# patrickfrey/strusPattern

Measured on AMD Instinct MI355X. Metric: GB/s input text scanned + matches/s, 10k-regex lexer + 10k-rule automaton, higher is better.
Workload: dtype u64; 1 GPU; configs[4] per-GPU shard: 10001 regexes + 10000 token rules, 12288 docs x 64KiB UTF-8 per step (the same 805 MB resident in HBM every step; configs[4] asks 32 GB per GPU: 39 such steps)

## Files before the change

### struspattern_amd/csrc/l2_fast.h

```cpp
#ifndef SPA_L2_FAST_H
#define SPA_L2_FAST_H
#include <stdint.h>
#include <string>
#include <vector>
#include "l2_tables.h"
#include "l2_device.h"

namespace spa {

struct FastKeyInst
{
	uint32_t resultHandle;
	uint32_t formatHandle;
	uint32_t pastEvent;
	uint32_t meta;
	struct { uint32_t event; uint32_t info; } trig[ 3];
	uint32_t hw0;
	uint32_t ranksA;
	uint32_t ranksB;
	uint32_t totals;
	uint32_t items;
	uint32_t flags;
};
enum {
// ... 68 lines not shown
	{
		s.count = 0; s.value = 0; s.flags |= S_DEL;
		return;
	}
	if (took)
	{
		if ((info & FTI_HASVAR) && withItems)
		{
			const uint32_t item = elex | ((info >> FTI_VAR_SHIFT) << 24);
			if ((s.flags & S_DONE) && !(s.flags & S_HASLIST)) {}
			else if (s.nItems == 0) { s.it0 = item; s.nItems = 1; }
			else if (s.nItems == 1) { s.it1 = item; s.nItems = 2; }
			else if (s.nItems == 2) { s.it2 = item; s.nItems = 3; }
			else s.flags |= S_ODD;
		}
		if (!(s.flags & S_HASSTART)) { s.startLex = elex; s.flags |= S_TOOK; if (esord) s.flags |= S_HASSTART; }
	}
	if (m)
	{
		if (!(s.flags & S_DONE)) { s.flags |= S_DONE | S_RESULT; if (s.nItems) s.flags |= S_HASLIST; }
		if (f) s.flags |= S_FIN;
	}
}

struct FastKeyEntry
{
	uint32_t event;
	uint32_t kiBegin;
	uint32_t kiCount;
	uint32_t stopIdx;
};

enum {FAST_LISTCAP=64, FAST_EXPCAP=1024, FAST_MAXSTOP=64, FAST_SPILL_BUCKET=1024, FAST_VARIANTS=5, FAST_RQCAP=192};

struct FastSpillLayout
{
	uint32_t maxRules;
	uint32_t oCold;
	uint32_t oHot, oLink;
	uint32_t oKi, oLex0;
	uint32_t oFree;
	uint32_t oEnt;
	uint32_t oStaged;
	uint32_t maxStaged;
	uint32_t oList;
	uint32_t oExp;
	uint32_t totalWords;
};

enum {SPD_FAST_FALLBACK=100};

struct FastParams
{
	const FastKeyInst* keyinst;
	const FastStatic* statics;
	const FastKeyEntry* keytab;
	uint32_t keymask;
	uint32_t nofStopWords;
	uint32_t expShift;
	uint32_t bucketMeta[ 16];
	FastSpillLayout spill;
	uint32_t* spillBase;
	uint32_t* fallbackList; uint32_t* fallbackCount;
	uint32_t* diag;
	L2BatchIO io;
	uint64_t* prof;
// ... 15 lines not shown
```

### struspattern_amd/csrc/l2_fast_kernel.hip

```cpp
#include <hip/hip_runtime.h>
#include <stdint.h>
#include "l2_fast.h"
#include "l2_device.h"
#include "wave_scan.h"

using namespace spa;

namespace {

typedef uint16_t u16;
typedef uint8_t u8;

typedef const __attribute__((address_space(4))) FastParams& KP;
__device__ __forceinline__ KP kernelParams() { return *(const __attribute__((address_space(4))) FastParams*)__builtin_amdgcn_kernarg_segment_ptr(); }

#define WAVE_FENCE() __builtin_amdgcn_fence( __ATOMIC_ACQ_REL, "wavefront")

enum {NIL16=0xFFFFu};

#ifdef SPA_PROF
#define PROF_DECL u64 prof_t0 = __builtin_amdgcn_s_memtime()
#define PROF_ADD( SLOT) do { const u64 prof_t1 = __builtin_amdgcn_s_memtime(); w.prof[ SLOT] += prof_t1 - prof_t0; prof_t0 = prof_t1; } while (0)
#else
#define PROF_DECL do {} while (0)
// ... 40 lines not shown
{
	const u32 inc = 1u << ((h & 3u)*8), ws = h >> 2;
	c0 += ws == 0 ? inc : 0u; c1 += ws == 1 ? inc : 0u; c2 += ws == 2 ? inc : 0u; c3 += ws == 3 ? inc : 0u;
}

#define FALLBACK( WHY) do { w.err = SPD_FAST_FALLBACK; w.why = (WHY); } while (0)
enum {FB_LEXEMS=1, FB_DISPOSE=2, FB_ITEM_AFTER_RESULT=3, FB_ITEMS=4, FB_STAGED=5, FB_RULES=8, FB_BUCKET_SIZE=9, FB_POSLEXEMS=10};

__device__ __forceinline__ bool endLE( u32 hw, u32 pos) { return (hw & H_ENDZERO) || ((hw >> H_END_SHIFT) & H_END_MASK) != ((pos + 1u) & 0xFFu); }
__device__ __forceinline__ bool endEQ( u32 hw, u32 pos) { return (hw & H_ENDZERO) ? (pos == 0) : (((hw >> H_END_SHIFT) & H_END_MASK) == (pos & 0xFFu)); }
__device__ __forceinline__ u32 withEnd( u32 hw, u32 end) { return (hw & ~((H_END_MASK << H_END_SHIFT) | H_ENDZERO)) | ((end & 0xFFu) << H_END_SHIFT); }

template <bool SMALL> struct FreeId { typedef u8 type; };
template <> struct FreeId<false> { typedef u16 type; };
template <int R, int T>
struct LdsDoc
{
	u32 hot[ R];
	u32 kl[ R];
	u64 ent[ T];
	u32 bsize[ 16];
	u32 bmeta[ 16];
	u16 link[ 3*R];
	typename FreeId<(R <= 256)>::type freeS[ R];
	u16 exp[ FAST_EXPCAP];
	u16 expCnt[ 64];
	u16 list[ FAST_LISTCAP];
	u16 rq[ FAST_RQCAP];
};

struct Wave
{
	u32* sp;
	u32 curpos, timestamp, nInstalled, nAlt, nSignals, nTrig, openLo, openHi;
	u32 freeN, usedL, sFreeN, usedS;
	u32 nDispose, nStaged, nStagedItems, err;
	u32 lbase;
	u32 spill;
	u32 why;
	u32 posLexems;
	u32 stopLex, stopOrd, stopTs;
	u32 bsizeV, bmetaV;
	u32 expCntV;
#ifdef SPA_PROF
	u64 prof[ 12];
#endif
};

template <int R, int T>
struct Engine
{
typedef LdsDoc<R,T> Lds;
typedef __attribute__((address_space(3))) Lds& LR;

template <bool SP> static __device__ __forceinline__ u32 ldHot( LR L, const Wave& w, KP P, u32 r) { if (!SP || r < (u32)R) return L.hot[ r]; return w.sp[ P.spill.oHot + (r - R)]; }
template <bool SP> static __device__ __forceinline__ void stHot( LR L, const Wave& w, KP P, u32 r, u32 v) { if (!SP || r < (u32)R) L.hot[ r] = v; else w.sp[ P.spill.oHot + (r - R)] = v; }
template <bool SP> static __device__ __forceinline__ u32 ldLink( LR L, const Wave& w, KP P, u32 r, u32 j) { if (!SP || r < (u32)R) return (u32)L.link[ 3*r + j]; return w.sp[ P.spill.oLink + 3*(r - R) + j]; }
template <bool SP> static __device__ __forceinline__ void stLink( LR L, const Wave& w, KP P, u32 r, u32 j, u32 v) { if (!SP || r < (u32)R) L.link[ 3*r + j] = (u16)v; else w.sp[ P.spill.oLink + 3*(r - R) + j] = v; }
template <bool SP> static __device__ __forceinline__ void ldLinks( LR L, const Wave& w, KP P, u32 r, u32& l0, u32& l1, u32& l2)
{
	if (!SP || r < (u32)R) { l0 = (u32)L.link[ 3*r]; l1 = (u32)L.link[ 3*r+1]; l2 = (u32)L.link[ 3*r+2]; }
	else { const u32* q = &w.sp[ P.spill.oLink + 3*(r - R)]; l0 = q[0]; l1 = q[1]; l2 = q[2]; }
}
template <bool SP> static __device__ __forceinline__ u32 ldKl( LR L, const Wave& w, KP P, u32 r) { if (!SP || r < (u32)R) return L.kl[ r]; return w.sp[ P.spill.oKi + (r - R)]; }
template <bool SP> static __device__ __forceinline__ void stKl( LR L, const Wave& w, KP P, u32 r, u32 ki, u32 lx)
{ const u32 v = ki | (lx << 20); if (!SP || r < (u32)R) L.kl[ r] = v; else w.sp[ P.spill.oKi + (r - R)] = v; }
static __device__ __forceinline__ u32 keyLexemOf( u32 kl, u32 lbase) { return lbase - ((lbase - (kl >> 20)) & 0xFFFu); }
template <bool SP> static __device__ __forceinline__ u32 ldExp( LR L, const Wave& w, KP P, u32 row, u32 i)
{ const u32 C = (u32)FAST_EXPCAP >> P.expShift; if (!SP || i < C) return (u32)L.exp[ row*C + i]; return w.sp[ P.spill.oExp + row*P.spill.maxRules + (i - C)]; }
template <bool SP> static __device__ __forceinline__ void stExp( LR L, const Wave& w, KP P, u32 row, u32 i, u32 r)
{ const u32 C = (u32)FAST_EXPCAP >> P.expShift; if (!SP || i < C) L.exp[ row*C + i] = (u16)r; else w.sp[ P.spill.oExp + row*P.spill.maxRules + (i - C)] = r; }
template <bool SP> static __device__ __forceinline__ u32 ldEv( LR L, const Wave& w, KP P, u32 h, u32 meta, u32 pos)
{ if (!SP || pos < (meta >> 16)) return (u32)L.ent[ (meta & 0xFFFFu) + pos]; return w.sp[ P.spill.oEnt + 2*(h*FAST_SPILL_BUCKET + pos - (meta >> 16))]; }
template <bool SP> static __device__ __forceinline__ uint2 ldEnt( LR L, const Wave& w, KP P, u32 h, u32 meta, u32 pos)
{ if (!SP || pos < (meta >> 16)) { const u64 v = L.ent[ (meta & 0xFFFFu) + pos]; return make_uint2( (u32)v, (u32)(v >> 32)); } return *(const uint2*)&w.sp[ P.spill.oEnt + 2*(h*FAST_SPILL_BUCKET + pos - (meta >> 16))]; }
template <bool SP> static __device__ __forceinline__ u32 ldTs( LR L, const Wave& w, KP P, u32 h, u32 meta, u32 pos) { return ldEnt<SP>( L, w, P, h, meta, pos).y; }
template <bool SP> static __device__ __forceinline__ void stEnt( LR L, const Wave& w, KP P, u32 h, u32 meta, u32 pos, u32 e, u32 t)
{
	if (!SP || pos < (meta >> 16)) L.ent[ (meta & 0xFFFFu) + pos] = (u64)e | ((u64)t << 32);
	else *(uint2*)&w.sp[ P.spill.oEnt + 2*(h*FAST_SPILL_BUCKET + pos - (meta >> 16))] = make_uint2( e, t);
}
template <bool SP> static __device__ __forceinline__ u32 ldList( LR L, const Wave& w, KP P, u32 i) { if (!SP || i < (u32)FAST_LISTCAP) return (u32)L.list[ i]; return w.sp[ P.spill.oList + i]; }
static __device__ __forceinline__ void pushList( LR L, Wave& w, KP P, u32 i, u32 r)
{
	if (i < (u32)FAST_LISTCAP) { if (LANE == 0) L.list[ i] = (u16)r; }
	else { w.spill = 1; if (LANE == 0) w.sp[ P.spill.oList + i] = r; }
}

enum {STAGED_LINE=0x80000000u};
static __device__ __forceinline__ void stageLineResult( Wave& w, KP P, u32 at, u32 ki, u32 startLex, u32 endLex, u32 nStatic, u32 hasNew, u32 newVar, u32 keyLex)
{
	u32* S = &w.sp[ P.spill.oStaged + 8*at];
	st4( S, (u32)STAGED_LINE | ki, 0u, startLex, endLex);
	*(uint2*)(S+4) = make_uint2( nStatic | (hasNew << 2) | (newVar << 8), keyLex);
}
static __device__ __forceinline__ void stageResult( Wave& w, KP P, u32 at, u32 handle, u32 fmt, u32 startLex, u32 endLex, u32 nItems, u32 vars, u32 i0, u32 i1, u32 i2)
{
	u32* S = &w.sp[ P.spill.oStaged + 8*at];
	st4( S, handle, fmt, startLex, endLex);
	st4( S+4, nItems | (vars << 8), i0, i1, i2);
}

template <bool SP>
static __device__ __forceinline__ void fireSignal( LR L, Wave& w, KP P, u32 tsv, u32 sord)
{
	const u32 tid = tsv & 0xFFFFu, r = tid >> 2;
	const u32 sigval = (tsv >> 16) & 0xFu, sigtype = (tsv >> 20) & 0x7u, hasVar = (tsv >> 23) & 1u, variable = tsv >> 24;
	u32 hw = uni( ldHot<SP>( L, w, P, r));
	w.nSignals += 1;
	u32 value = hw & H_VALUE_MASK, count = (hw >> H_COUNT_SHIFT) & H_COUNT_MASK;
	bool match = false, take = false, fin = false;
	switch (sigtype)
	{
		case SIG_ANY:
			take = true;
			if (count > 0) { match = true; --count; fin = (count == 0); hw = withEnd( hw, sord+1); }
			break;
		case SIG_SEQUENCE:
		case SIG_SEQUENCE_IMM:
			if (sigval == value && (sigtype == SIG_SEQUENCE ? endLE( hw, sord) : endEQ( hw, sord)))
			{
				hw = withEnd( hw, sord+1); value = sigval-1;
				if (count > 0) { --count; match = (count == 0); } else match = true;
				fin = (value == 0); take = true;
			}
			break;
		case SIG_WITHIN:
			if ((sigval & value) != 0 && endLE( hw, sord))
			{
				hw = withEnd( hw, sord+1); value &= ~sigval;
				if (count > 0) { --count; match = (count == 0); } else match = true;
				take = true;
			}
			break;
		default:
			hw &= ~(H_VALUE_MASK | (H_COUNT_MASK << H_COUNT_SHIFT));
			if (!(hw & H_LISTED))
			{
				if (w.nDispose < P.spill.maxRules) { pushList( L, w, P, w.nDispose, r); w.nDispose += 1; hw |= H_LISTED; } else FALLBACK( FB_DISPOSE);
			}
			if (LANE == 0) stHot<SP>( L, w, P, r, hw);
			return;
// ... 157 lines not shown
			handle = c0.x; fmt = c0.y; startLex = c0.z; it0 = c0.w; it1 = c1.x; it2 = c1.y;
		}
		else
		{
			const u32* K = (const u32*)&P.keyinst[ kl & 0xFFFFFu];
			handle = K[ 0]; fmt = K[ 1];
			const u32 vars = K[ 14];
			startLex = lx;
			it0 = lx | ((vars & 0xFFu) << 24); it1 = lx | (((vars >> 8) & 0xFFu) << 24); it2 = lx | (((vars >> 16) & 0xFFu) << 24);
		}
		if (newItem)
		{
			const u32 item = w.lbase | (variable << 24);
			if (nItems == 0) it0 = item; else if (nItems == 1) it1 = item; else it2 = item;
			nItemsOut = nItems + 1u;
		}
		if (newStart) startLex = w.lbase;
	}
	else if (lineCase && newItem) nItemsOut = nItems + 1u;
	const bool resLine = lineCase && (hw & H_VISIBLE) != 0, resRec = recCase && match && handle != 0;
	const u64 resM = __ballot( resLine || resRec);
	const u32 nres = (u32)__popcll( resM);
	const bool listNow = hit && !(hw & H_LISTED) && (isDel || (match && fin));
	const u64 listM = __ballot( listNow);
	const u32 nlist = (u32)__popcll( listM);
	{
		const u64 whyM = __ballot( why != 0);
		u32 fb = 0;
		if (whyM) fb = (u32)__builtin_amdgcn_readlane( why, (u32)__builtin_ctzll( whyM));
		else if (w.nStaged + nres > P.spill.maxStaged) fb = FB_STAGED;
		else if (w.nDispose + nlist > P.spill.maxRules) fb = FB_DISPOSE;
		if (fb) { FALLBACK( fb); return true; }
	}
	w.nSignals += nh;
	if (nres)
	{
		const u32 at = w.nStaged + (u32)__popcll( resM & lanesBelow());
		if (resLine) stageLineResult( w, P, at, kl & 0xFFFFFu, newStart ? w.lbase : lx, w.lbase, nItems, newItem ? 1u : 0u, variable, lx);
		if (resRec)
		{
			const u32 ia = nItemsOut == 3 ? it2 : nItemsOut == 2 ? it1 : it0;
			const u32 ib = nItemsOut == 3 ? it1 : it0;
			const u32 ic = it0;
			const u32 vars = nItemsOut == 0 ? 0u : nItemsOut == 1 ? (ia >> 24) : nItemsOut == 2 ? ((ia >> 24) | ((ib >> 24) << 8)) : ((ia >> 24) | ((ib >> 24) << 8) | ((ic >> 24) << 16));
			stageResult( w, P, at, handle, fmt, startLex, w.lbase, nItemsOut, vars, ia & 0xFFFFFFu, ib & 0xFFFFFFu, ic & 0xFFFFFFu);
		}
		w.nStaged += nres;
		const u32 itemsIncl = waveScanAdd( (resLine || resRec) ? nItemsOut : 0u);
		w.nStagedItems += (u32)__builtin_amdgcn_readlane( itemsIncl, 63);
	}
	if (recCase && !match)
	{
		st4( cold, handle, fmt, startLex, it0); *(uint2*)(cold + 4) = make_uint2( it1, it2);
		hw |= H_COLD;
	}
	if (nlist)
	{
		if (listNow) L.list[ w.nDispose + (u32)__popcll( listM & lanesBelow())] = (u16)r;
		w.nDispose += nlist;
	}
	if (hit)
	{
		if (listNow) hw |= H_LISTED;
		if (!isDel)
		{
			if (newStart && sord) hw |= H_HASSTART;
			hw = (hw & ~(H_VALUE_MASK | (H_COUNT_MASK << H_COUNT_SHIFT) | (H_NITEMS_MASK << H_NITEMS_SHIFT))) | value | (count << H_COUNT_SHIFT) | ((live ? nItemsOut : nItems) << H_NITEMS_SHIFT);
// ... 18 lines not shown
#if defined(SPA_PROF) && !defined(SPA_PROF_INSTALL)
		u64 pd0 = __builtin_amdgcn_s_memtime();
#define PROF_D( SLOT) do { if (__ballot( hw == 0xFFFFFFFFu)) w.err = SPD_ERR_INTERNAL; const u64 pd1 = __builtin_amdgcn_s_memtime(); w.prof[ SLOT] += pd1 - pd0; pd0 = pd1; } while (0)
#else
#define PROF_D( SLOT) do {} while (0)
#endif
		if (have)
		{
			r = isExp ? ldExp<SP>( L, w, P, row, nE - 1u - (base + LANE - nD)) : ldList<SP>( L, w, P, base + LANE);
			hw = ldHot<SP>( L, w, P, r);
		}
		const bool act = have && (hw & H_ACTIVE) && !(isExp && (hw & H_LISTED));
		const u32 mask = act ? ((hw >> H_TMASK_SHIFT) & H_TMASK_MASK) : 0u;
		if (act) stHot<SP>( L, w, P, r, hw & ~(H_ACTIVE | (H_TMASK_MASK << H_TMASK_SHIFT)));
		if (__ballot( mask != 0))
		{
			u32 lk[ 3] = {0,0,0};
			if (mask) ldLinks<SP>( L, w, P, r, lk[ 0], lk[ 1], lk[ 2]);
#if defined(SPA_PROF) && !defined(SPA_PROF_INSTALL)
			if (__ballot( lk[ 0] == 0xFFFFFFFFu)) w.err = SPD_ERR_INTERNAL;
#endif
			PROF_D( 6);
			const bool slot2 = __ballot( (mask & 4u) != 0) != 0;
			u32 c0 = 0, c1 = 0, c2 = 0, c3 = 0;
#pragma unroll
			for (int j=0; j<2; ++j) if ((mask >> j) & 1u) byteInc( c0, c1, c2, c3, lk[ j] >> 12);
			if (slot2) { if (mask & 4u) byteInc( c0, c1, c2, c3, lk[ 2] >> 12); }
			const u32 i0 = waveScanAdd( c0), i1 = waveScanAdd( c1), i2 = waveScanAdd( c2), i3 = waveScanAdd( c3);
			const u32 e0 = i0 - c0, e1 = i1 - c1, e2 = i2 - c2, e3 = i3 - c3;
			const u32 t0 = (u32)__builtin_amdgcn_readlane( i0, 63), t1 = (u32)__builtin_amdgcn_readlane( i1, 63);
			const u32 t2 = (u32)__builtin_amdgcn_readlane( i2, 63), t3 = (u32)__builtin_amdgcn_readlane( i3, 63);
			const u32 tot = LANE < 16u ? byteField( t0, t1, t2, t3, LANE) : 0u;
			const u32 qoff = waveScanAdd( tot) - tot;
			const u32 total = (u32)__builtin_amdgcn_readlane( qoff + tot, 15);
			if (slot2)
			{
				const u32 h = lk[ 2] >> 12;
				const u32 qo = (u32)__builtin_amdgcn_ds_bpermute( (int)(h << 2), (int)qoff);
				if (mask & 4u) L.rq[ qo + byteField( e0, e1, e2, e3, h)] = (u16)(4u*r + 2u);
			}
#pragma unroll
			for (int j=1; j>=0; --j)
			{
				const u32 h = lk[ j] >> 12;
				const u32 qo = (u32)__builtin_amdgcn_ds_bpermute( (int)(h << 2), (int)qoff);
				if ((mask >> j) & 1u)
				{
					u32 mineBefore = 0;
					if (slot2 && (mask & 4u) && (lk[ 2] >> 12) == h) ++mineBefore;
					if (j == 0 && (mask & 2u) && (lk[ 1] >> 12) == h) ++mineBefore;
					L.rq[ qo + byteField( e0, e1, e2, e3, h) + mineBefore] = (u16)(4u*r + (u32)j);
				}
			}
			WAVE_FENCE();
			PROF_D( 7);
			if (LANE < 16u && tot)
			{
				const u32 h = LANE, meta = w.bmetaV;
				u32 size = w.bsizeV;
				u32 tidNext = (u32)L.rq[ qoff];
				for (u32 q=0; q<tot; ++q)
				{
					const u32 tid = tidNext;
					{ const u32 nx = qoff + q + 1u; tidNext = (u32)L.rq[ nx < (u32)FAST_RQCAP ? nx : (u32)FAST_RQCAP - 1u]; }
					const u32 pos = ldLink<SP>( L, w, P, tid >> 2, tid & 3u) & 0xFFFu;
					const u32 last = size - 1u;
					const uint2 m = ldEnt<SP>( L, w, P, h, meta, last);
					if (!SP || pos != last)
					{
						stEnt<SP>( L, w, P, h, meta, pos, m.x, m.y);
						stLink<SP>( L, w, P, (m.y & 0xFFFFu) >> 2, m.y & 3u, (h << 12) | pos);
					}
					size = last;
					if (SP) WAVE_FENCE();
				}
				L.bsize[ h] = size;
				w.bsizeV = size;
			}
			WAVE_FENCE();
			PROF_D( 11);
			w.nTrig -= total;
#ifdef SPA_PROF
			w.prof[ 8] += (u32)__builtin_amdgcn_readlane( waveScanMax( tot), 63); w.prof[ 9] += 1; w.prof[ 10] += nb;
#endif
		}
		if (nE)
		{
			const bool fr = have && isExp;
			const u64 mL = __ballot( fr && r < (u32)R);
			if (fr && r < (u32)R) L.freeS[ w.freeN + (u32)__popcll( mL & lanesBelow())] = (typename FreeId<(R <= 256)>::type)r;
			w.freeN += (u32)__popcll( mL);
			if (SP)
			{
				const u64 mS = __ballot( fr && r >= (u32)R);
				if (fr && r >= (u32)R) w.sp[ P.spill.oFree + w.sFreeN + (u32)__popcll( mS & lanesBelow())] = r - R;
				w.sFreeN += (u32)__popcll( mS);
			}
		}
		WAVE_FENCE();
	}
}

static __device__ __forceinline__ void setCurrentPos( LR L, Wave& w, KP P, u32 pos)
{
	const u32 W = 1u << P.expShift;
	u32 wcnt = 0;
	while (!w.err)
	{
		u32 n = 0, row = 0;
		while (wcnt < W && w.curpos < pos && !n)
		{
			row = w.curpos & (W-1u);
			n = (u32)__builtin_amdgcn_readlane( w.expCntV, row);
			++wcnt; ++w.curpos;
// ... 59 lines not shown
	for (int j=0; j<3; ++j)
	{
		hB[ j] = (tInfo[ j] >> FTI_BUCKET_SHIFT) & 15u;
		inst[ j] = mat && (tInfo[ j] & FTI_INSTALL);
		if (inst[ j]) byteInc( c0, c1, c2, c3, hB[ j]);
	}
	u32 tmask = 0;
	if (__ballot( inst[ 0] || inst[ 1] || inst[ 2]))
	{
		u32 i0 = waveScanAdd( c0), i1 = waveScanAdd( c1), i2 = waveScanAdd( c2), i3 = waveScanAdd( c3);
		const u32 e0 = i0 - c0, e1 = i1 - c1, e2 = i2 - c2, e3 = i3 - c3;
		const u32 t0 = (u32)__builtin_amdgcn_readlane( i0, 63), t1 = (u32)__builtin_amdgcn_readlane( i1, 63);
		const u32 t2 = (u32)__builtin_amdgcn_readlane( i2, 63), t3 = (u32)__builtin_amdgcn_readlane( i3, 63);
		u32 oldSize = 0, add = 0;
		if (LANE < 16u) { oldSize = L.bsize[ LANE]; add = byteField( t0, t1, t2, t3, LANE); }
#pragma unroll
		for (int j=0; j<3; ++j)
		{
			if (inst[ j])
			{
				const u32 h = hB[ j];
				u32 sameB = 0;
#pragma unroll
				for (int jj=0; jj<j; ++jj) if (inst[ jj] && hB[ jj] == h) ++sameB;
				const u32 pos = L.bsize[ h] + byteField( e0, e1, e2, e3, h) + sameB;
				const u32 sv = (tInfo[ j] & FTI_SIGVAL_MASK) | (((tInfo[ j] >> FTI_SIGTYPE_SHIFT) & FTI_SIGTYPE_MASK) << 4) | ((tInfo[ j] & FTI_HASVAR) ? 0x80u : 0u);
				stEnt<SP>( L, w, P, h, L.bmeta[ h], pos, tEv[ j], (4*r + (u32)j) | (sv << 16) | ((tInfo[ j] >> FTI_VAR_SHIFT) << 24));
				stLink<SP>( L, w, P, r, (u32)j, (h << 12) | pos);
				tmask |= 1u << j;
			}
		}
		WAVE_FENCE();
		if (LANE < 16u && add) L.bsize[ LANE] = oldSize + add;
		{
			const u32 s = t0 + t1 + t2 + t3;
			w.nTrig += (s & 0xFFu) + ((s >> 8) & 0xFFu) + ((s >> 16) & 0xFFu) + (s >> 24);
		}
	}
	if (mat)
	{
		u32 hw = value | (count << H_COUNT_SHIFT) | H_ACTIVE | H_COLD | (tmask << H_TMASK_SHIFT) | (nItems << H_NITEMS_SHIFT);
		hw |= end ? ((end & 0xFFu) << H_END_SHIFT) : (u32)H_ENDZERO;
		if (done) hw |= H_DONE;
		if (hasStart) hw |= H_HASSTART;
		if (del || fin) hw |= H_LISTED;
		stHot<SP>( L, w, P, r, hw);
		u32* cold = &w.sp[ P.spill.oCold + 8*r];
		st4( cold, handle, fmt, startLex, it0);
		*(uint2*)(cold + 4) = make_uint2( it1, it2);
	}
	{
		const bool emit = have && resultNow && handle != 0;
		const u64 rm = __ballot( emit);
		if (rm)
		{
			const u32 nr = (u32)__popcll( rm);
			if (w.nStaged + nr > P.spill.maxStaged) { FALLBACK( FB_STAGED); return; }
			if (emit)
			{
				const u32 ia = nItems == 3 ? it2 : nItems == 2 ? it1 : it0;
				const u32 ib = nItems == 3 ? it1 : it0;
				const u32 ic = it0;
				const u32 vars = nItems == 0 ? 0u : nItems == 1 ? (ia >> 24) : nItems == 2 ? ((ia >> 24) | ((ib >> 24) << 8)) : ((ia >> 24) | ((ib >> 24) << 8) | ((ic >> 24) << 16));
				stageResult( w, P, w.nStaged + (u32)__popcll( rm & lanesBelow()), handle, fmt, startLex, w.lbase, nItems, vars, ia & 0xFFFFFFu, ib & 0xFFFFFFu, ic & 0xFFFFFFu);
			}
			w.nStaged += nr;
			u32 incl = waveScanAdd( emit ? nItems : 0u);
			w.nStagedItems += (u32)__builtin_amdgcn_readlane( incl, 63);
		}
	}
// ... 60 lines not shown
		}
		u32 hw = (hw0 & ~(H_NITEMS_MASK << H_NITEMS_SHIFT)) | (nItems << H_NITEMS_SHIFT);
		hw |= (fl & FKF_END_SET) ? (((sord + 1u) & 0xFFu) << H_END_SHIFT) : (u32)H_ENDZERO;
		stHot<SP>( L, w, P, r, hw);
		stKl<SP>( L, w, P, r, ki0 + LANE, w.lbase);
	}
	const u32 nres = (totals >> 16) & 0xFFu;
	if (nres)
	{
		if (w.nStaged + nres > P.spill.maxStaged) { FALLBACK( FB_STAGED); return; }
		if (have && (fl & FKF_RESULT_NOW))
		{
			const u32 v0 = q3.z & 0xFFu, v1 = (q3.z >> 8) & 0xFFu, v2 = (q3.z >> 16) & 0xFFu;
			const u32 va = nItems == 3 ? v2 : nItems == 2 ? v1 : v0;
			const u32 vb = nItems == 3 ? v1 : v0;
			const u32 vars = nItems == 0 ? 0u : nItems == 1 ? va : nItems == 2 ? (va | (vb << 8)) : (va | (vb << 8) | (v0 << 16));
			stageResult( w, P, w.nStaged + ((ranksA >> 16) & 0xFFu), handle, fmt, (fl & FKF_START_SET) ? w.lbase : 0u, w.lbase, nItems, vars, w.lbase, w.lbase, w.lbase);
		}
		w.nStaged += nres;
		if (P.io.withItems) w.nStagedItems += itemsTotal;
	}
	const u32 nd = totals >> 24;
	if (nd)
	{
		if (w.nDispose + nd > P.spill.maxRules) { FALLBACK( FB_DISPOSE); return; }
		if (w.nDispose + nd > (u32)FAST_LISTCAP) w.spill = 1;
		if (have && (fl & FKF_DISPOSE_NOW))
		{
			const u32 at = w.nDispose + (ranksA >> 24);
			if (at < (u32)FAST_LISTCAP) L.list[ at] = (u16)r; else w.sp[ P.spill.oList + at] = r;
		}
		w.nDispose += nd;
	}
	w.nTrig += totals & 0xFFu;
	WAVE_FENCE();
}

static __device__ __forceinline__ bool allocRuleIds( LR L, Wave& w, KP P, u64 matMask, u32& r)
{
	const bool mat = (matMask >> LANE) & 1ull;
	const u32 nmat = (u32)__popcll( matMask);
	const u32 rank = (u32)__popcll( matMask & lanesBelow());
	r = 0;
	if (nmat)
	{
		const u32 a = w.freeN < nmat ? w.freeN : nmat;
		const u32 roomL = (u32)R - w.usedL;
		const u32 b = (nmat - a) < roomL ? (nmat - a) : roomL;
		const u32 rest = nmat - a - b;
		if (rest)
		{
			const u32 c = w.sFreeN < rest ? w.sFreeN : rest;
			const u32 d = rest - c;
			if ((u32)R + w.usedS + d > P.spill.maxRules) { FALLBACK( FB_RULES); return false; }
			w.spill = 1;
			if (mat && rank >= a+b)
			{
				if (rank < a+b+c) r = (u32)R + w.sp[ P.spill.oFree + w.sFreeN - 1 - (rank - a - b)];
				else r = (u32)R + w.usedS + (rank - a - b - c);
			}
			w.sFreeN -= c; w.usedS += d;
		}
		if (mat)
		{
			if (rank < a) r = (u32)L.freeS[ w.freeN - 1 - rank];
			else if (rank < a+b) r = w.usedL + (rank - a);
		}
// ... 58 lines not shown
	const u32 nItems = P.io.withItems ? ((hw0 >> H_NITEMS_SHIFT) & H_NITEMS_MASK) : 0u;
	if (have)
	{
		const u32 close = (misc >> FSM_EXPCLOSE_SHIFT) & 0xFFu;
		if (close) L.expCnt[ row] = (u16)(cnt + close);
#pragma unroll
		for (int t=0; t<2; ++t) if (info[ t] & FSI_LAST) L.bsize[ (info[ t] >> FSI_BUCKET_SHIFT) & 15u] = oldB[ t] + ((info[ t] >> FSI_RANK_SHIFT) & 0xFFu) + 1u;
		u32 hw = (hw0 & ~(H_NITEMS_MASK << H_NITEMS_SHIFT)) | (nItems << H_NITEMS_SHIFT);
		hw |= (misc & FSM_END_SET) ? (((sord + 1u) & 0xFFu) << H_END_SHIFT) : (u32)H_ENDZERO;
		stHot<SP>( L, w, P, r, hw);
		stKl<SP>( L, w, P, r, ki0 + LANE, w.lbase);
	}
	const u32 nres = (totals >> 16) & 0xFFu;
	if (nres)
	{
		if (w.nStaged + nres > P.spill.maxStaged) { FALLBACK( FB_STAGED); return; }
		if (have && (misc & FSM_RESULT_NOW))
			stageLineResult( w, P, w.nStaged + (ranks & 0xFFu), ki0 + LANE, (misc & FSM_START_SET) ? w.lbase : 0u, w.lbase, nItems, 0u, 0u, w.lbase);
		w.nStaged += nres;
		if (P.io.withItems) w.nStagedItems += itemsTotal;
	}
	const u32 nd = totals >> 24;
	if (nd)
	{
		if (w.nDispose + nd > P.spill.maxRules) { FALLBACK( FB_DISPOSE); return; }
		if (w.nDispose + nd > (u32)FAST_LISTCAP) w.spill = 1;
		if (have && (misc & FSM_DISPOSE_NOW))
		{
			const u32 at = w.nDispose + ((ranks >> 8) & 0xFFu);
			if (at < (u32)FAST_LISTCAP) L.list[ at] = (u16)r; else w.sp[ P.spill.oList + at] = r;
		}
		w.nDispose += nd;
	}
	w.nTrig += totals & 0xFFu;
	w.nSignals += (totals >> 8) & 0xFFu;
	WAVE_FENCE();
}

static __device__ __forceinline__ void installBatch( LR L, Wave& w, KP P, u32 kb, u32 kc, u32 sord, const uint4 pc0, const uint4 pc1)
{
	for (u32 base=0; base<kc && !w.err; base+=64)
	{
		const u32 nb = (kc - base) < 64u ? (kc - base) : 64u;
		const bool have = LANE < nb;
		uint4 c0 = pc0, c1 = pc1;
		if (base)
		{
			c0 = make_uint4( 0,0,0,0); c1 = c0;
			if (have) { const u32* S = (const u32*)&P.statics[ kb + base + LANE]; c0 = ld4( S); c1 = ld4( S+4); }
		}
#ifdef SPA_PROF_INSTALL
		u64 pi0 = __builtin_amdgcn_s_memtime();
#define PROF_I( SLOT, V) do { if (__ballot( (V) == 0xFFFFFFF1u)) w.err = SPD_ERR_INTERNAL; const u64 pi1 = __builtin_amdgcn_s_memtime(); w.prof[ SLOT] += pi1 - pi0; pi0 = pi1; } while (0)
#else
#define PROF_I( SLOT, V) do {} while (0)
#endif
		if ((uni( c1.y) & FSM_BATCH_COMPACT) && sord != 0)
		{
			PROF_I( 6, c1.y);
			const u32 info[ 2] = {c0.y, c0.w};
			const u32 row = (sord + (c1.y & FSM_RANGE_MASK)) & ((1u << P.expShift) - 1u);
			u32 cnt = 0, oldB[ 2] = {0,0}, metaB[ 2] = {0,0};
			bool inst[ 3] = {false,false,false}; u32 hB[ 3] = {0,0,0};
			if (have)
			{
				cnt = (u32)L.expCnt[ row];
#pragma unroll
				for (int t=0; t<2; ++t)
// ... 52 lines not shown
#pragma unroll
					for (int j=2; j>=0; --j)
					{
						if ((tInfo[ j] & FTI_INSTALL) && tEv[ j] == pastEvent) fireLocal( sim, tInfo[ j], psord, plex, P.io.withItems);
					}
					bool cancelled = false;
#pragma unroll
					for (int j=0; j<3; ++j)
					{
						if ((tInfo[ j] & FTI_INSTALL) && ((tInfo[ j] >> FTI_SIGTYPE_SHIFT) & FTI_SIGTYPE_MASK) == SIG_DEL)
						{
							const u32 ts = delTs[ j];
							if (ts && ts > pts) cancelled = true;
						}
					}
					if (cancelled || (sim.flags & (S_DEL | S_FIN))) dropped = true;
				}
			}
			w.nAlt += (u32)__popcll( __ballot( have && pastEvent != 0));
		}
		if (!isStatic)
		{
			if (have && !dropped)
			{
#pragma unroll
				for (int j=0; j<3; ++j) if (tInfo[ j] & FTI_KEY) fireLocal( sim, tInfo[ j], sord, w.lbase, P.io.withItems);
			}
			if (__ballot( (sim.flags & S_ODD) != 0)) { FALLBACK( FB_ITEMS); return; }
		}
		const bool mat = have && !dropped;
		const u64 matMask = __ballot( mat);
		const u32 nmat = (u32)__popcll( matMask);
		w.nInstalled += nb;
		if (isStatic) w.nSignals += (uni( q3.y) >> 8) & 0xFFu;
		else
		{
			u32 incl = waveScanAdd( have ? sim.nFires : 0u);
			w.nSignals += (u32)__builtin_amdgcn_readlane( incl, 63);
		}
		u32 r;
		if (!allocRuleIds( L, w, P, matMask, r)) return;
		if (nmat && !w.spill)
		{
			const u32 row = (sord + range) & ((1u << P.expShift) - 1u);
			const bool over = mat && (u32)L.expCnt[ row] + nmat > ((u32)FAST_EXPCAP >> P.expShift);
			if (__ballot( over)) w.spill = 1;
		}
		{
			bool inst[ 3]; u32 hB[ 3];
#pragma unroll
			for (int j=0; j<3; ++j) { inst[ j] = mat && (tInfo[ j] & FTI_INSTALL); hB[ j] = (tInfo[ j] >> FTI_BUCKET_SHIFT) & 15u; }
			if (!checkBuckets( L, w, P, isStatic ? (uni( q3.y) & 0xFFu) : 3*nmat, inst, hB)) return;
		}
		if (isStatic)
		{
			if (w.spill) installStaticT<true>( L, w, P, kb + base, nb, sord, r, q0, q1, q2, q3);
			else installStaticT<false>( L, w, P, kb + base, nb, sord, r, q0, q1, q2, q3);
		}
		else if (w.spill) installBatchT<true>( L, w, P, kb, nb, sord, matMask, r, q0, q1, q2, sim);
		else installBatchT<false>( L, w, P, kb, nb, sord, matMask, r, q0, q1, q2, sim);
		w.bsizeV = L.bsize[ LANE & 15u];
	}
	w.bsizeV = L.bsize[ LANE & 15u];
	w.expCntV = (u32)L.expCnt[ LANE];
}

template <bool SP>
static __device__ __forceinline__ void scanAndFire( LR L, Wave& w, KP P, u32 id, u32 ordpos)
{
	const u32 h = evhash( id) & 15u;
	const u32 n = (u32)__builtin_amdgcn_readlane( w.bsizeV, h);
	const u32 meta = (u32)__builtin_amdgcn_readlane( w.bmetaV, h);
	for (u32 base=0; base<n && !w.err; base+=64)
	{
		const u32 i = base + LANE;
		uint2 en = make_uint2( 0, 0);
		if (i < n) en = ldEnt<SP>( L, w, P, h, meta, i);
		u64 m = __ballot( i < n && en.x == id);
		if (!SP && (m & (m - 1ull)) != 0)
		{
			if (fireBatch( L, w, P, m, en.y, ordpos)) m = 0;
		}
		while (m && !w.err)
		{
			const u32 p = (u32)__builtin_ctzll( m);
			m &= m-1;
			const u32 tsv = (u32)__builtin_amdgcn_readlane( en.y, p);
			fireSignal<SP>( L, w, P, tsv, ordpos);
		}
	}
}

static __device__ __forceinline__ void runKernel()
{
	KP P = kernelParams();
	__shared__ Lds ldsDoc;
	LR L = *(__attribute__((address_space(3))) Lds*)&ldsDoc;
	Wave w;
	w.sp = P.spillBase + (u64)blockIdx.x * P.spill.totalWords;
	const u32 ndocs = P.io.ndocs;
	const u32 waveSlot = blockIdx.x, nWaveSlots = gridDim.x;

	for (u32 round=0; round<=ndocs; ++round)
	{
		u32 doc = waveSlot;
		if (round)
		{
			u32 nx = 0;
			if (LANE == 0) nx = atomicAdd( P.io.docCursor, 1u);
			doc = nWaveSlots + uni( nx);
		}
		if (doc >= ndocs) break;
		w.bmetaV = P.bucketMeta[ LANE & 15u]; w.bsizeV = 0; w.expCntV = 0;
		if (LANE < 16u) { L.bsize[ LANE] = 0; L.bmeta[ LANE] = w.bmetaV; }
		L.expCnt[ LANE] = 0;
		w.stopLex = 0; w.stopOrd = 0; w.stopTs = 0; w.posLexems = 0;
		w.curpos = 0; w.timestamp = 0; w.nInstalled = 0; w.nAlt = 0; w.nSignals = 0; w.nTrig = 0; w.openLo = 0; w.openHi = 0;
		w.freeN = 0; w.usedL = 0; w.sFreeN = 0; w.usedS = 0;
		w.nDispose = 0; w.nStaged = 0; w.nStagedItems = 0; w.err = 0; w.lbase = 0; w.why = 0; w.spill = 0;
#ifdef SPA_PROF
		for (int pi=0; pi<12; ++pi) w.prof[ pi] = 0;
#endif
		WAVE_FENCE();

		u64 lbeg, lend;
		docLexems( P.io, doc, lbeg, lend);
		if (lend - lbeg >= (1ull << 24)) FALLBACK( FB_LEXEMS);
		u32 curPosition = 0, nEvents = 0;
		for (u64 tile=lbeg; tile<lend && !w.err; tile+=64)
		{
			PROF_DECL;
			uint4 lx = make_uint4( 0,0,0,0); u32 seg = 0;
			const bool mine = tile + LANE < lend;
			if (mine)
			{
				lx = ((const uint4*)P.io.lexems)[ tile + LANE];
				if (P.io.origseg) seg = P.io.origseg[ tile + LANE];
			}
			u32 kBegin = 0, kCount = 0, kStop = 0;
			if (mine && lx.x && lx.x < (1u<<29))
			{
				u32 slot = keyHash( lx.x) & P.keymask;
				for (u32 probes=0; probes<=P.keymask; ++probes)
				{
					const uint4 eq = ld4( &P.keytab[ slot]);
					if (eq.x == lx.x) { kBegin = eq.y; kCount = eq.z; kStop = eq.w; break; }
					if (eq.x == 0) break;
					slot = (slot+1) & P.keymask;
				}
			}
			const u32 cnt = (lend - tile) < 64 ? (u32)(lend - tile) : 64u;
#ifdef SPA_PROF
			if (__ballot( kBegin == 0xFFFFFFFFu)) break;
#endif
			PROF_ADD( 5);
			for (u32 k=0; k<cnt && !w.err; ++k)
			{
				const u32 id = __builtin_amdgcn_readlane( lx.x, k), ordpos = __builtin_amdgcn_readlane( lx.y, k);
				const u32 origpos = __builtin_amdgcn_readlane( lx.z, k), origsize = __builtin_amdgcn_readlane( lx.w, k);
				const u32 origseg = __builtin_amdgcn_readlane( seg, k);
				if (curPosition > ordpos) { w.err = SPD_ERR_ORDER; break; }
				else if (curPosition < ordpos) { curPosition = ordpos; w.posLexems = 0; }
				else if (origsize >= 0x7FFFFFFFu || origseg >= 0x7FFFFFFFu || origpos >= 0x7FFFFFFFu) { w.err = SPD_ERR_RANGE; break; }
				if (w.curpos != ordpos || w.nDispose) { setCurrentPos( L, w, P, ordpos); PROF_ADD( 3); if (w.err) break; }
				if (id >= (1u<<29)) { w.err = SPD_ERR_RANGE; break; }
				w.lbase = (u32)(tile - lbeg) + k;
				if (++w.posLexems > 60u) { FALLBACK( FB_POSLEXEMS); break; }
				{
					const u32 lo = w.openLo + w.nTrig;
					if (lo < w.openLo) w.openHi += 1;
					w.openLo = lo;
				}
				const u32 kb = __builtin_amdgcn_readlane( kBegin, k), kc = __builtin_amdgcn_readlane( kCount, k);
				const u32 stopIdx = __builtin_amdgcn_readlane( kStop, k);
				uint4 pc0 = make_uint4( 0,0,0,0), pc1 = pc0;
				if (LANE < kc) { const u32* S = (const u32*)&P.statics[ kb + LANE]; pc0 = ld4( S); pc1 = ld4( S+4); }
				if (id)
				{
					if (w.spill) scanAndFire<true>( L, w, P, id, ordpos); else scanAndFire<false>( L, w, P, id, ordpos);
				}
				PROF_ADD( 0);
				if (w.err) break;
				if (kc) installBatch( L, w, P, kb, kc, ordpos, pc0, pc1);
				PROF_ADD( 1);
				if (w.err) break;
				WAVE_FENCE();
				if (stopIdx)
				{
					if (LANE == stopIdx-1u) { w.stopLex = w.lbase; w.stopOrd = ordpos; w.stopTs = w.timestamp + 1u; }
					w.timestamp += 1;
					WAVE_FENCE();
				}
				PROF_ADD( 2);
				++nEvents;
			}
		}

		PROF_DECL;
		u32 nres = w.err ? 0 : w.nStaged;
		const u32 nitems = (w.err || !P.io.withItems) ? 0 : w.nStagedItems;
		u64 resBase = 0, itemBase = 0;
		if (nres && !reserveOutput( P.io, SPC_RESULTS, nres, resBase)) { w.err = SPD_ERR_OUTPUT; nres = 0; }
		if (nres && nitems && !reserveOutput( P.io, SPC_ITEMS, nitems, itemBase)) { w.err = SPD_ERR_OUTPUT; nres = 0; }
		if (nres)
		{
// ... 28 lines not shown
				}
				const u32 ni = P.io.withItems ? (s1.x & 0xFFu) : 0u;
				u32 incl = waveScanAdd( ni);
				const u64 mine = ip + (incl - ni);
				if (hv)
				{
					const uint4 a = ((const uint4*)P.io.lexems)[ lbeg + s0.z], z = ((const uint4*)P.io.lexems)[ lbeg + s0.w];
					const u32 sa = P.io.origseg ? P.io.origseg[ lbeg + s0.z] : 0u, sz = P.io.origseg ? P.io.origseg[ lbeg + s0.w] : 0u;
					u32* o = P.io.results + (resBase + ri)*9;
					o[0] = s0.x; o[1] = a.y; o[2] = z.y + 1u; o[3] = sa; o[4] = a.z; o[5] = sz; o[6] = z.z + z.w;
					o[7] = P.io.withItems ? (u32)mine : 0u; o[8] = ni;
					if (P.io.withFormats) P.io.resultFormat[ resBase + ri] = s0.y;
					const u32 il[ 3] = {s1.y, s1.z, s1.w};
#pragma unroll
					for (int q=0; q<3; ++q)
					{
						if ((u32)q < ni)
						{
							const uint4 t = ((const uint4*)P.io.lexems)[ lbeg + il[ q]];
							const u32 st = P.io.origseg ? P.io.origseg[ lbeg + il[ q]] : 0u;
							u32* io = P.io.items + (mine + (u32)q)*7;
							io[0] = (s1.x >> (8 + 8*q)) & 0xFFu; io[1] = t.y; io[2] = t.y + 1u; io[3] = st; io[4] = t.z; io[5] = st; io[6] = t.z + t.w;
							if (P.io.withFormats) { P.io.itemFormat[ 2*(mine + (u32)q)] = 0; P.io.itemFormat[ 2*(mine + (u32)q)+1] = 0; }
						}
					}
				}
				ip += (u32)__builtin_amdgcn_readlane( incl, 63);
			}
		}
		PROF_ADD( 4);
#ifdef SPA_PROF
		if (LANE == 0 && P.prof) for (int pi=0; pi<12; ++pi) atomicAdd( (unsigned long long*)&P.prof[ pi], (unsigned long long)w.prof[ pi]);
#endif
		if (w.err != SPD_FAST_FALLBACK) finishDocument( P.io, doc, resBase, nres, w.nInstalled, w.nAlt, w.nSignals, ((u64)w.openHi << 32) | w.openLo, w.err, nEvents);
		else if (LANE == 0)
		{
			const u32 at = atomicAdd( P.fallbackCount, 1u);
			P.fallbackList[ at] = doc;
			P.io.docRange[ 2*(u64)doc] = 0; P.io.docRange[ 2*(u64)doc+1] = 0;
			P.io.docStatus[ doc] = (int32_t)SPD_FAST_FALLBACK;
			atomicAdd( (unsigned long long*)&P.io.counters[ SPC_HANDOVER], 1ull);
			if (P.diag) { atomicAdd( &P.diag[ 0], 1u); atomicAdd( &P.diag[ w.why & 15u], 1u); }
		}
	}
}
};

}

#ifndef SPA_L2_FAST_WAVES_PER_EU
#define SPA_L2_FAST_WAVES_PER_EU 4
#endif
#define SPA_L2_FAST_OCC __attribute__((amdgpu_waves_per_eu( SPA_L2_FAST_WAVES_PER_EU, SPA_L2_FAST_WAVES_PER_EU)))
#define SPA_FAST_VARIANTS( V) \
	V( s, 192, 312) \
	V( m, 320, 512) \
	V( l, 512, 1024) \
	V( t, 8, 128)		 \
	V( n, 256, 448)
#define SPA_FAST_INSTANCE( X, RR, TT) \
	extern "C" __global__ __launch_bounds__(64) SPA_L2_FAST_OCC void spa_l2_fast_kernel_##X( FastParams kernelArgs) { Engine<RR,TT>::runKernel(); }
SPA_FAST_VARIANTS( SPA_FAST_INSTANCE)

namespace spa {
struct FastVariant { void (*kernel)( FastParams); uint32_t R, T; const char* name; };
#define SPA_FAST_ENTRY( X, RR, TT) {spa_l2_fast_kernel_##X, RR, TT, "spa_l2_fast_kernel_" #X},
static const FastVariant fastVariants[ FAST_VARIANTS] = { SPA_FAST_VARIANTS( SPA_FAST_ENTRY) };
// ... 23 lines not shown
```

Before: 4.247 GB/s.

## Defer signal and open-trigger counters to per-lane accumulators folded at flush

Replaces the scalar nSignals and nTrig bookkeeping with per-lane accumulators. Signals are now counted per lane from hit masks and fire counts. The open-trigger sum is derived from the per-bucket sizes (bsizeV) added once per lexem, instead of tracking nTrig increments and decrements everywhere. Partial sums are reduced with wave scans only every FAST_OPEN_FLUSH lexems and at document end. This removes several per-event wave reductions and scalar updates from the hot loop, at the risk of subtle mismatches in the reported statistics if bsizeV does not exactly equal the old nTrig.

```diff
diff --git a/struspattern_amd/csrc/l2_fast.h b/struspattern_amd/csrc/l2_fast.h
--- a/struspattern_amd/csrc/l2_fast.h
+++ b/struspattern_amd/csrc/l2_fast.h
@@ -124,6 +124,7 @@
 };
 
 enum {FAST_LISTCAP=64, FAST_EXPCAP=1024, FAST_MAXSTOP=64, FAST_SPILL_BUCKET=1024, FAST_VARIANTS=5, FAST_RQCAP=192};
+enum {FAST_OPEN_FLUSH=32768};
 
 struct FastSpillLayout
 {
diff --git a/struspattern_amd/csrc/l2_fast_kernel.hip b/struspattern_amd/csrc/l2_fast_kernel.hip
--- a/struspattern_amd/csrc/l2_fast_kernel.hip
+++ b/struspattern_amd/csrc/l2_fast_kernel.hip
@@ -96,7 +96,8 @@
 struct Wave
 {
 	u32* sp;
-	u32 curpos, timestamp, nInstalled, nAlt, nSignals, nTrig, openLo, openHi;
+	u32 curpos, timestamp, nInstalled, nAlt;
+	u32 openLo, openHi;
 	u32 freeN, usedL, sFreeN, usedS;
 	u32 nDispose, nStaged, nStagedItems, err;
 	u32 lbase;
@@ -106,6 +107,8 @@
 	u32 stopLex, stopOrd, stopTs;
 	u32 bsizeV, bmetaV;
 	u32 expCntV;
+	u32 nSignalsV;
+	u32 openV;
 #ifdef SPA_PROF
 	u64 prof[ 12];
 #endif
@@ -171,7 +174,6 @@
 	const u32 tid = tsv & 0xFFFFu, r = tid >> 2;
 	const u32 sigval = (tsv >> 16) & 0xFu, sigtype = (tsv >> 20) & 0x7u, hasVar = (tsv >> 23) & 1u, variable = tsv >> 24;
 	u32 hw = uni( ldHot<SP>( L, w, P, r));
-	w.nSignals += 1;
 	u32 value = hw & H_VALUE_MASK, count = (hw >> H_COUNT_SHIFT) & H_COUNT_MASK;
 	bool match = false, take = false, fin = false;
 	switch (sigtype)
@@ -395,7 +397,6 @@
 		else if (w.nDispose + nlist > P.spill.maxRules) fb = FB_DISPOSE;
 		if (fb) { FALLBACK( fb); return true; }
 	}
-	w.nSignals += nh;
 	if (nres)
 	{
 		const u32 at = w.nStaged + (u32)__popcll( resM & lanesBelow());
@@ -480,7 +481,6 @@
 			const u32 t2 = (u32)__builtin_amdgcn_readlane( i2, 63), t3 = (u32)__builtin_amdgcn_readlane( i3, 63);
 			const u32 tot = LANE < 16u ? byteField( t0, t1, t2, t3, LANE) : 0u;
 			const u32 qoff = waveScanAdd( tot) - tot;
-			const u32 total = (u32)__builtin_amdgcn_readlane( qoff + tot, 15);
 			if (slot2)
 			{
 				const u32 h = lk[ 2] >> 12;
@@ -527,7 +527,6 @@
 			}
 			WAVE_FENCE();
 			PROF_D( 11);
-			w.nTrig -= total;
 #ifdef SPA_PROF
 			w.prof[ 8] += (u32)__builtin_amdgcn_readlane( waveScanMax( tot), 63); w.prof[ 9] += 1; w.prof[ 10] += nb;
 #endif
@@ -653,10 +652,6 @@
 		}
 		WAVE_FENCE();
 		if (LANE < 16u && add) L.bsize[ LANE] = oldSize + add;
-		{
-			const u32 s = t0 + t1 + t2 + t3;
-			w.nTrig += (s & 0xFFu) + ((s >> 8) & 0xFFu) + ((s >> 16) & 0xFFu) + (s >> 24);
-		}
 	}
 	if (mat)
 	{
@@ -783,7 +778,6 @@
 		}
 		w.nDispose += nd;
 	}
-	w.nTrig += totals & 0xFFu;
 	WAVE_FENCE();
 }
 
@@ -908,8 +902,7 @@
 		}
 		w.nDispose += nd;
 	}
-	w.nTrig += totals & 0xFFu;
-	w.nSignals += (totals >> 8) & 0xFFu;
+	w.nSignalsV += LANE == 0 ? ((totals >> 8) & 0xFFu) : 0u;
 	WAVE_FENCE();
 }
 
@@ -1028,12 +1021,8 @@
 		const u64 matMask = __ballot( mat);
 		const u32 nmat = (u32)__popcll( matMask);
 		w.nInstalled += nb;
-		if (isStatic) w.nSignals += (uni( q3.y) >> 8) & 0xFFu;
-		else
-		{
-			u32 incl = waveScanAdd( have ? sim.nFires : 0u);
-			w.nSignals += (u32)__builtin_amdgcn_readlane( incl, 63);
-		}
+		if (isStatic) w.nSignalsV += LANE == 0 ? ((uni( q3.y) >> 8) & 0xFFu) : 0u;
+		else w.nSignalsV += have ? sim.nFires : 0u;
 		u32 r;
 		if (!allocRuleIds( L, w, P, matMask, r)) return;
 		if (nmat && !w.spill)
@@ -1072,7 +1061,9 @@
 		const u32 i = base + LANE;
 		uint2 en = make_uint2( 0, 0);
 		if (i < n) en = ldEnt<SP>( L, w, P, h, meta, i);
-		u64 m = __ballot( i < n && en.x == id);
+		const bool hit = i < n && en.x == id;
+		u64 m = __ballot( hit);
+		w.nSignalsV += hit ? 1u : 0u;
 		if (!SP && (m & (m - 1ull)) != 0)
 		{
 			if (fireBatch( L, w, P, m, en.y, ordpos)) m = 0;
@@ -1085,6 +1076,16 @@
 			fireSignal<SP>( L, w, P, tsv, ordpos);
 		}
 	}
+}
+
+static __device__ __forceinline__ void foldOpen( Wave& w)
+{
+	const bool bucketLane = LANE < 16u;
+	const u32 lo16 = (u32)__builtin_amdgcn_readlane( waveScanAdd( bucketLane ? (w.openV & 0xFFFFu) : 0u), 63);
+	const u32 hi16 = (u32)__builtin_amdgcn_readlane( waveScanAdd( bucketLane ? (w.openV >> 16) : 0u), 63);
+	const u64 sum = (((u64)w.openHi << 32) | w.openLo) + ((u64)hi16 << 16) + lo16;
+	w.openLo = (u32)sum; w.openHi = (u32)(sum >> 32);
+	w.openV = 0;
 }
 
 static __device__ __forceinline__ void runKernel()
@@ -1111,7 +1112,7 @@
 		if (LANE < 16u) { L.bsize[ LANE] = 0; L.bmeta[ LANE] = w.bmetaV; }
 		L.expCnt[ LANE] = 0;
 		w.stopLex = 0; w.stopOrd = 0; w.stopTs = 0; w.posLexems = 0;
-		w.curpos = 0; w.timestamp = 0; w.nInstalled = 0; w.nAlt = 0; w.nSignals = 0; w.nTrig = 0; w.openLo = 0; w.openHi = 0;
+		w.curpos = 0; w.timestamp = 0; w.nInstalled = 0; w.nAlt = 0; w.nSignalsV = 0; w.openV = 0; w.openLo = 0; w.openHi = 0;
 		w.freeN = 0; w.usedL = 0; w.sFreeN = 0; w.usedS = 0;
 		w.nDispose = 0; w.nStaged = 0; w.nStagedItems = 0; w.err = 0; w.lbase = 0; w.why = 0; w.spill = 0;
 #ifdef SPA_PROF
@@ -1146,6 +1147,7 @@
 				}
 			}
 			const u32 cnt = (lend - tile) < 64 ? (u32)(lend - tile) : 64u;
+			if (((u32)(tile - lbeg) & ((u32)FAST_OPEN_FLUSH - 1u)) == 0) foldOpen( w);
 #ifdef SPA_PROF
 			if (__ballot( kBegin == 0xFFFFFFFFu)) break;
 #endif
@@ -1162,11 +1164,7 @@
 				if (id >= (1u<<29)) { w.err = SPD_ERR_RANGE; break; }
 				w.lbase = (u32)(tile - lbeg) + k;
 				if (++w.posLexems > 60u) { FALLBACK( FB_POSLEXEMS); break; }
-				{
-					const u32 lo = w.openLo + w.nTrig;
-					if (lo < w.openLo) w.openHi += 1;
-					w.openLo = lo;
-				}
+				w.openV += w.bsizeV;
 				const u32 kb = __builtin_amdgcn_readlane( kBegin, k), kc = __builtin_amdgcn_readlane( kCount, k);
 				const u32 stopIdx = __builtin_amdgcn_readlane( kStop, k);
 				uint4 pc0 = make_uint4( 0,0,0,0), pc1 = pc0;
@@ -1261,7 +1259,12 @@
 #ifdef SPA_PROF
 		if (LANE == 0 && P.prof) for (int pi=0; pi<12; ++pi) atomicAdd( (unsigned long long*)&P.prof[ pi], (unsigned long long)w.prof[ pi]);
 #endif
-		if (w.err != SPD_FAST_FALLBACK) finishDocument( P.io, doc, resBase, nres, w.nInstalled, w.nAlt, w.nSignals, ((u64)w.openHi << 32) | w.openLo, w.err, nEvents);
+		if (w.err != SPD_FAST_FALLBACK)
+		{
+			const u32 nSignals = (u32)__builtin_amdgcn_readlane( waveScanAdd( w.nSignalsV), 63);
+			foldOpen( w);
+			finishDocument( P.io, doc, resBase, nres, w.nInstalled, w.nAlt, nSignals, ((u64)w.openHi << 32) | w.openLo, w.err, nEvents);
+		}
 		else if (LANE == 0)
 		{
 			const u32 at = atomicAdd( P.fallbackCount, 1u);
```

New measurement: 4.096 GB/s. 3.6% lower.
